# dpeerlab/segger

Hardware: AMD Instinct MI355X
Metric: edges scored/sec (tx->cell) fwd+bwd (higher is better)
Workload: dtype bf16; 1 GPU; C2: single Xenium-scale tile per GPU, 1000000 tx, 10000 nuclei, k=15 kNN (Ett=15000000, Etb=393796, Ep=2435646), training step fwd+bwd+Adam, attention dropout 0.2; parallelism=dp1

## Files before the change

include/segger_amd.h:

```cpp
#ifndef SEGGER_AMD_H
#define SEGGER_AMD_H

#include <stddef.h>
#include <stdint.h>

#ifdef __cplusplus
extern "C" {
#endif

#if defined(__GNUC__) || defined(__clang__)
#pragma GCC visibility push(default)
#endif

#define SEGGER_ABI_VERSION 32

enum segger_status {
  SEGGER_OK = 0,
  SEGGER_EINVAL = -1,
  SEGGER_EUNSUPPORTED = -2,
  SEGGER_EHIP = -3,
  SEGGER_EWORKSPACE = -4
};

enum segger_dtype { SEGGER_F32 = 0, SEGGER_BF16 = 1, SEGGER_F16 = 2 };
// ... 256 lines not shown
int segger_sample_negatives(const int64_t* pos, int64_t n, int64_t n_b, const int64_t* n_b_dev, uint64_t seed,
                            const uint64_t* seed_dev, int64_t* neg, segger_stream_t stream);

int segger_metric_fwd(const void* z, int64_t ld_z, int64_t n, int32_t channels, int32_t dtype, const int64_t* pos,
                      const int64_t* neg, const float* d_pos, const float* d_neg, const float* w, float eps,
                      float* loss, void* workspace, size_t workspace_bytes, segger_stream_t stream);
int segger_metric_bwd(const void* z, int64_t ld_z, int64_t n, int32_t channels, int32_t dtype, const int64_t* pos,
                      const int64_t* neg, const float* d_pos, const float* d_neg, const float* w, float eps,
                      const float* grad_scale_dev, float* grad_z, segger_stream_t stream);

size_t segger_triplet_workspace_bytes(int64_t n_edges);
int segger_triplet_fwd(const segger_triplet_args* args, segger_stream_t stream);
int segger_triplet_bwd(const segger_triplet_args* args, segger_stream_t stream);

#define SEGGER_LOSS_HEAD_DEFER_FINISH 1
typedef struct segger_loss_head_args {
  const void* z_tx; int64_t ld_ztx; int64_t n_tx;
  const void* z_bd; int64_t ld_zbd; int64_t n_bd;
  int32_t channels, dtype;
  const int64_t* tx_pos; const int64_t* tx_neg; float tx_margin, tx_eps;
  const int64_t* bd_pos; const int64_t* bd_neg; const float* bd_dpos; const float* bd_dneg; const float* bd_w; float bd_eps;
  int32_t sg_kind;
  const int64_t* sg_src; const int64_t* sg_pos; const int64_t* sg_neg; int64_t n_sg; float sg_margin, sg_eps;
  const int64_t* sg_pos_indptr; const int32_t* sg_pos_eid; const int32_t* sg_of_tx;
  const float* a; const float* b; const float* grad_out; float* out; float* grad_raw;
  float* tx_w; int32_t* tx_state; int32_t* tx_next; int32_t* tx_hot_id; float* tx_hot_acc;
  const void* y_tx; int64_t ld_ytx; float norm_eps; int32_t reserved_;
  void* grad_tx; int64_t ld_gtx; float* grad_bd;
  void* workspace; size_t workspace_bytes; int32_t* ticket;
} segger_loss_head_args;
size_t segger_loss_head_workspace_bytes(int64_t n_tx, int64_t n_bd, int64_t n_sg);
int64_t segger_loss_head_max_hot_rows(int64_t n_tx);
int segger_loss_head_supported(int32_t channels, int32_t dtype);
int segger_loss_head_fwd(const segger_loss_head_args* args, segger_stream_t stream);
int segger_loss_head_bwd(const segger_loss_head_args* args, segger_stream_t stream);

#define SEGGER_MINMAX_INITIALISED 1
#define SEGGER_MINMAX_KEEP_EMPTY 2
int segger_segment_minmax_ex(const float* pos, const int64_t* batch, int64_t n, int64_t n_graphs, float* mins, float* maxs,
                             int32_t flags, segger_stream_t stream);
int segger_segment_minmax(const float* pos, const int64_t* batch, int64_t n, int64_t n_graphs,
                          float* mins, float* maxs, segger_stream_t stream);

int segger_linear_supported(int32_t k_in, int32_t m_out, int32_t dtype);
int segger_linear_fwd(const void* x, int64_t ldx, const void* w, const float* bias, void* y, int64_t ldy,
                      int64_t n_rows, int32_t k_in, int32_t m_out, int32_t dtype, segger_stream_t stream);
int segger_linear_fwd_silu_grad(const void* x, int64_t ldx, const void* w, const void* gate, int64_t ld_gate, void* y,
// ... 277 lines not shown
```

segger_amd/_lib.py:

```python
from __future__ import annotations

import ctypes as C
import os
from typing import Optional

import torch

_HERE = os.path.dirname(os.path.abspath(__file__))
LIB_PATH = os.environ.get("SEGGER_AMD_LIB") or os.path.join(_HERE, "libsegger_amd.so")
ABI_VERSION = 32
THRESHOLDS_CHUNK = 1024
FEATURES_TILE, FEATURES_SLAB_ROWS, FEATURES_MAX_SLABS = 64, 512, 32
FEATURES_MAX_COLS, FEATURES_MAX_K = 32768, 256
KNN_BF_MAX_D, KNN_BF_MAX_K, KNN_BF_MAX_SLABS = 256, 64, 32
CONTAM_MAX_TYPES, CONTAM_MAX_K, CONTAM_MAX_REF_GENES, CONTAM_LDS_BYTES = 256, 64, 32768, 65536
MORPH_MAX_VERTS, MORPH_COLS, MORPH_ERR_OFFSETS, MORPH_ERR_CAP = 4096, 12, 1, 2
PJOIN_CONTAINS, PJOIN_INTERSECTS = 0, 1
PJOIN_ERR_OFFSETS, PJOIN_ERR_CAP, PJOIN_ERR_BUFFER, PJOIN_ERR_FILL = 1, 2, 4, 8
BOUNDARY_MAX_SMOOTHING, BOUNDARY_CHUNK_MAX_HULL, BOUNDARY_COUNTERS = 6, 2048, 8
OUTLINE_MAX_POINTS, OUTLINE_COUNTERS = 2048, 10

SEGGER_F32, SEGGER_BF16, SEGGER_F16 = 0, 1, 2
DTYPE_CODE = {torch.float32: SEGGER_F32, torch.bfloat16: SEGGER_BF16, torch.float16: SEGGER_F16}

# ... 147 lines not shown


class FrontJoinArgs(C.Structure):
    _fields_ = [
        ("table", vp), ("ids", vp), ("n_rows_table", C.c_int32), ("D", C.c_int32), ("dtype", C.c_int32), ("reserved_", C.c_int32),
        ("pe", vp), ("ld_pe", C.c_int64), ("n_tx", C.c_int64), ("n_bd", C.c_int64),
        ("xb", vp), ("ld_xb", C.c_int64),
        ("out_tx", vp), ("ld_out_tx", C.c_int64), ("out_bd", vp), ("ld_out_bd", C.c_int64),
        ("g_tx", vp), ("ld_g_tx", C.c_int64), ("g_bd", vp), ("ld_g_bd", C.c_int64),
        ("g_pe", vp), ("ld_g_pe", C.c_int64), ("g_xb", vp), ("ld_g_xb", C.c_int64),
        ("g_table", vp), ("gene_ptr", vp), ("gene_rows", vp), ("workspace", vp), ("workspace_bytes", C.c_size_t),
    ]


LOSS_HEAD_DEFER_FINISH = 1


class LossHeadArgs(C.Structure):
    _fields_ = [
        ("z_tx", vp), ("ld_ztx", C.c_int64), ("n_tx", C.c_int64),
        ("z_bd", vp), ("ld_zbd", C.c_int64), ("n_bd", C.c_int64),
        ("channels", C.c_int32), ("dtype", C.c_int32),
        ("tx_pos", vp), ("tx_neg", vp), ("tx_margin", C.c_float), ("tx_eps", C.c_float),
        ("bd_pos", vp), ("bd_neg", vp), ("bd_dpos", vp), ("bd_dneg", vp), ("bd_w", vp), ("bd_eps", C.c_float),
        ("sg_kind", C.c_int32),
        ("sg_src", vp), ("sg_pos", vp), ("sg_neg", vp), ("n_sg", C.c_int64), ("sg_margin", C.c_float), ("sg_eps", C.c_float),
        ("sg_pos_indptr", vp), ("sg_pos_eid", vp), ("sg_of_tx", vp),
        ("a", vp), ("b", vp), ("grad_out", vp), ("out", vp), ("grad_raw", vp),
        ("tx_w", vp), ("tx_state", vp), ("tx_next", vp), ("tx_hot_id", vp), ("tx_hot_acc", vp),
        ("y_tx", vp), ("ld_ytx", C.c_int64), ("norm_eps", C.c_float), ("reserved_", C.c_int32),
# ... 106 lines not shown
    "segger_front_join_fwd": (C.c_int, [C.POINTER(FrontJoinArgs), vp]),
    "segger_front_join_bwd": (C.c_int, [C.POINTER(FrontJoinArgs), vp]),
    "segger_embed_gelu_bwd_workspace_bytes": (C.c_size_t, [C.c_int64, C.c_int32, C.c_int32]),
    "segger_embed_gelu_bwd": (C.c_int, [vp, C.c_int64, vp, vp, C.c_int64, C.c_int64, C.c_int32, C.c_int32, vp, C.c_int64,
                                        vp, vp, vp, vp, C.c_size_t, C.c_int32, vp]),
    "segger_l2norm_fwd": (C.c_int, [vp, C.c_int64, C.c_int64, C.c_int32, C.c_float, vp, C.c_int64, C.c_int32, vp]),
    "segger_l2norm_bwd": (C.c_int, [vp, C.c_int64, vp, C.c_int64, C.c_int64, C.c_int32, C.c_float, vp, C.c_int64, C.c_int32, vp]),
    "segger_segment_rowsum_workspace_bytes": (C.c_size_t, [C.c_int64, C.c_int32, C.c_int32]),
    "segger_segment_rowsum": (C.c_int, [vp, C.c_int64, C.c_int64, C.c_int32, C.c_int32, vp, vp, C.c_int32, vp, vp,
                                        C.c_size_t, vp]),
    "segger_colsum_workspace_bytes": (C.c_size_t, [C.c_int64, C.c_int32]),
    "segger_colsum": (C.c_int, [vp, C.c_int64, C.c_int64, C.c_int32, C.c_int32, vp, vp, C.c_size_t, vp]),
    "segger_l2norm_many": (C.c_int, [C.POINTER(L2NormSeg), C.c_int32, C.c_int32, C.c_float, C.c_int32, vp]),
    "segger_loss_head_workspace_bytes": (C.c_size_t, [C.c_int64, C.c_int64, C.c_int64]),
    "segger_loss_head_max_hot_rows": (C.c_int64, [C.c_int64]),
    "segger_loss_head_supported": (C.c_int, [C.c_int32, C.c_int32]),
    "segger_loss_head_fwd": (C.c_int, [C.POINTER(LossHeadArgs), vp]),
    "segger_loss_head_bwd": (C.c_int, [C.POINTER(LossHeadArgs), vp]),
    "segger_knn_workspace_bytes": (C.c_size_t, [C.c_int64, C.c_int32, C.c_int32]),
    "segger_knn_grid": (C.c_int, [vp, C.c_int64, vp, C.c_int64, C.c_int32, C.c_float, C.c_float, C.c_float, C.c_float,
                                  C.c_int32, C.c_int32, vp, vp, vp, C.c_size_t, vp]),
    "segger_quadtree_workspace_bytes": (C.c_int64, [C.c_int64, C.c_int32, C.c_int64, C.c_int64]),
    "segger_quadtree_build": (C.c_int, [vp, C.c_int64, C.c_double, C.c_double, C.c_double, C.c_int32, C.c_int64, C.c_int64,
                                        vp, vp, vp, vp, vp, vp, vp, vp, C.c_size_t, vp]),
    "segger_quadtree_label": (C.c_int, [vp, C.c_int64, C.c_double, C.c_double, C.c_double, C.c_double, C.c_double, C.c_int32,
                                        vp, vp, vp, vp, C.c_int64, vp, vp]),
    "segger_assign_update": (C.c_int, [vp, vp, vp, vp, vp, C.c_int64, vp, vp, vp, vp, C.c_int64, vp]),
    "segger_assign_finalize": (C.c_int, [vp, C.c_int64, vp, vp, vp]),
    "segger_expression_workspace_bytes": (C.c_int64, [C.c_int64, C.c_int64, C.c_int64]),
    "segger_expression_build": (C.c_int, [vp, vp, vp, vp, vp, C.c_int64, C.c_int64, C.c_int64, vp, vp, vp, vp, vp, vp, vp, vp,
# ... 122 lines not shown
```

segger_amd/csrc/loss_head.hip:

```cpp
#include "common.h"
#include "post_common.h"

namespace segger {
namespace {

constexpr int kItemsPerBlock = 64;
constexpr int kChainCap = 64;
constexpr int32_t kOverflow = -2;

template <typename T, int CPL> struct Row;
template <int CPL> struct Row<float, CPL> {
  static __device__ __forceinline__ void load(const float* p, float (&f)[CPL]) {
    if constexpr (CPL == 2) { const float2 v = *reinterpret_cast<const float2*>(p); f[0] = v.x; f[1] = v.y; }
    else {
#pragma unroll
      for (int k = 0; k < CPL; k += 4) {
        const f32x4 v = *reinterpret_cast<const f32x4*>(p + k);
        f[k] = v.x; f[k + 1] = v.y; f[k + 2] = v.z; f[k + 3] = v.w;
      }
    }
  }
  static __device__ __forceinline__ void store(float* p, const float (&f)[CPL]) {
    if constexpr (CPL == 2) *reinterpret_cast<float2*>(p) = float2{f[0], f[1]};
    else {
// ... 37 lines not shown
  Vec8<f16_t>::unpack2(*reinterpret_cast<const uint32_t*>(p), a, b);
}

__device__ __forceinline__ float softplus_(float x) { return fmaxf(x, 0.f) + log1pf(__expf(-fabsf(x))); }
__device__ __forceinline__ float sigmoid_(float x) { return 1.0f / (1.0f + __expf(-x)); }

struct LossHeadParams {
  const void* ztx; int64_t ld_ztx; int64_t n_tx;
  const void* zbd; int64_t ld_zbd; int64_t n_bd;
  const int64_t* tx_pos; const int64_t* tx_neg; float tx_margin, tx_eps;
  const int64_t* bd_pos; const int64_t* bd_neg; const float* bd_dpos; const float* bd_dneg; const float* bd_w; float bd_eps;
  const int64_t* sg_src; const int64_t* sg_pos; const int64_t* sg_neg; int64_t n_sg; float sg_margin, sg_eps; int sg_kind;
  const int64_t* sg_indptr; const int32_t* sg_eid; const int32_t* sg_of_tx;
  const float* a; const float* b; const float* gout; float* out; float* graw;
  float* tx_w; int32_t* state; int32_t* next;
  int32_t* hot_id; float* hot_acc; int64_t max_hot;
  const void* ytx; int64_t ld_ytx; float norm_eps;
  void* gtx; int64_t ld_gtx; float* gbd;
  float* partial; int32_t* ticket;
  int nb_tx, nb_bd, nb_sg;
  int nb_sg_fin;
  int defer;
};

__device__ __forceinline__ float graw_of(const LossHeadParams& p, int i) {
  return p.defer ? (p.gout[3] * p.b[i] + p.gout[i]) * p.a[i] : p.graw[i];
}

template <typename T, int CPL>
__global__ __launch_bounds__(256) void loss_head_fwd_kernel(LossHeadParams p) {
// ... 21 lines not shown
      float sp = 0.f, sn = 0.f;
#pragma unroll
      for (int k = 0; k < CPL; ++k) {
        const float dp = a[k] - pp[k] + p.tx_eps, dn = a[k] - nn[k] + p.tx_eps;
        sp = fmaf(dp, dp, sp); sn = fmaf(dn, dn, sn);
      }
      sp = lane_block_sum<16>(sp); sn = lane_block_sum<16>(sn);
      const float dap = sqrtf(sp), dan = sqrtf(sn);
      const float l = dap - dan + p.tx_margin;
      if (ok && gl == 0) acc += fmaxf(l, 0.f);
      if (p.tx_w != nullptr && t < p.n_tx) {
        const bool active = ok && l > 0.f;
        const float wp = active && dap > 0.f ? 1.0f / dap : 0.f;
        const float wn = active && dan > 0.f ? 1.0f / dan : 0.f;
        if (gl < 2) {
          const float wk = gl == 0 ? wp : wn;
          const int64_t tgt = gl == 0 ? ip : in;
          const int32_t code = (int32_t)(2 * t + gl);
          p.tx_w[code] = wk;
          if (wk != 0.f) {
            const int32_t slot = atomicAdd(p.state + 2 * tgt + 1, 1);
            if (slot < kChainCap) {
              p.next[code] = atomicExch(p.state + 2 * tgt, code + 1);
            } else {
              p.next[code] = kOverflow;
              if (slot == kChainCap) {
                const int32_t hid = atomicAdd(p.state + 2 * p.n_tx, 1);
                if ((int64_t)hid < p.max_hot) {
                  float* acc_row = p.hot_acc + (int64_t)hid * C;
                  for (int k = 0; k < C; ++k) acc_row[k] = 0.f;
                  p.hot_id[p.n_tx + hid] = 0;
                  __threadfence();
                }
                p.hot_id[tgt] = hid;
              }
            }
          }
        }
      }
    }
  } else if (blk < p.nb_tx + p.nb_bd) {
    const int64_t base = (int64_t)(blk - p.nb_tx) * kItemsPerBlock;
#pragma unroll 1
    for (int q = wave * 4 + grp; q < kItemsPerBlock; q += 16) {
      const int64_t i = base + q;
      bool ok = i < p.n_bd;
      int64_t ip = ok ? p.bd_pos[i] : 0, in = ok ? p.bd_neg[i] : 0;
      const float w = ok ? p.bd_w[i] : 0.f;
      if ((uint64_t)ip >= (uint64_t)p.n_bd || (uint64_t)in >= (uint64_t)p.n_bd || w == 0.f) { ok = false; ip = in = 0; }
      const int64_t ii = ok ? i : 0;
      float x[CPL], yp[CPL], yn[CPL];
      Row<T, CPL>::load(zbd + ii * p.ld_zbd + c0, x);
// ... 98 lines not shown
__global__ __launch_bounds__(256) void loss_head_bwd_kernel(LossHeadParams p) {
  constexpr int C = 16 * CPL;
  const int lane = threadIdx.x & 63, wave = threadIdx.x >> 6;
  const int grp = lane >> 4, gl = lane & 15, c0 = gl * CPL;
  const int blk = blockIdx.x;
  const T* ztx = static_cast<const T*>(p.ztx);
  const T* zbd = static_cast<const T*>(p.zbd);
  if (p.defer && blk == p.nb_tx + p.nb_bd + p.nb_sg) {
    loss_head_finish_body(p);
    return;
  }
  if (blk < p.nb_tx) {
    const float sc_tx = p.n_tx > 0 ? graw_of(p, 0) / (float)p.n_tx : 0.f;
    const float sc_sg = p.n_sg > 0 ? graw_of(p, 2) * (p.sg_kind == SEGGER_LOSS_BCE ? 0.5f : 1.0f) / (float)p.n_sg : 0.f;
    const int64_t base = (int64_t)blk * kItemsPerBlock;
    auto finish_row = [&](int64_t row, float (&g)[CPL]) {
      if (p.ytx != nullptr) {
        float y[CPL];
        Row<T, CPL>::load(static_cast<const T*>(p.ytx) + row * p.ld_ytx + c0, y);
        float ss = 0.f;
#pragma unroll
        for (int k = 0; k < CPL; ++k) ss = fmaf(y[k], y[k], ss);
        const float nrm = sqrtf(lane_block_sum<16>(ss));
        const float inv = 1.0f / fmaxf(nrm, p.norm_eps);
        float dot = 0.f;
#pragma unroll
        for (int k = 0; k < CPL; ++k) dot = fmaf(y[k] * inv, g[k], dot);
        dot = lane_block_sum<16>(dot);
        if (nrm < p.norm_eps) dot = 0.f;
#pragma unroll
        for (int k = 0; k < CPL; ++k) g[k] = (g[k] - y[k] * inv * dot) * inv;
      }
      Row<T, CPL>::store(static_cast<T*>(p.gtx) + row * p.ld_gtx + c0, g);
    };
    auto hot_add = [&](int64_t row, const float (&g)[CPL]) {
      const int64_t hid = p.hot_id[row];
      if ((uint64_t)hid >= (uint64_t)p.max_hot) return;
      float* acc = p.hot_acc + hid * C + c0;
#pragma unroll
      for (int k = 0; k < CPL; ++k) atomicAdd(acc + k, g[k]);
      __threadfence();
      int32_t old = 0;
      if (gl == 0) old = atomicAdd(p.hot_id + p.n_tx + hid, 1);
      old = __shfl(old, lane & 48, 64);
      if (old == p.state[2 * row + 1] - kChainCap) {
        __threadfence();
        float t[CPL];
#pragma unroll
        for (int k = 0; k < CPL; ++k) t[k] = __hip_atomic_load(acc + k, __ATOMIC_RELAXED, __HIP_MEMORY_SCOPE_AGENT);
        finish_row(row, t);
      }
    };
#pragma unroll 1
    for (int i = wave * 4 + grp; i < kItemsPerBlock; i += 16) {
      const int64_t r = base + i;
      if (r >= p.n_tx) continue;
      float a[CPL], g[CPL];
      Row<T, CPL>::load(ztx + r * p.ld_ztx + c0, a);
#pragma unroll
      for (int k = 0; k < CPL; ++k) g[k] = 0.f;
      const float uwp = p.tx_w[2 * r], uwn = p.tx_w[2 * r + 1];
      const float wp = uwp * sc_tx, wn = uwn * sc_tx;
      if (uwp != 0.f || uwn != 0.f) {
        const int64_t ip = p.tx_pos[r], in = p.tx_neg[r];
        float pp[CPL], nn[CPL], dp[CPL], dn[CPL];
        Row<T, CPL>::load(ztx + ip * p.ld_ztx + c0, pp);
        Row<T, CPL>::load(ztx + in * p.ld_ztx + c0, nn);
#pragma unroll
        for (int k = 0; k < CPL; ++k) {
          dp[k] = (a[k] - pp[k] + p.tx_eps) * wp; dn[k] = (a[k] - nn[k] + p.tx_eps) * wn;
          g[k] += dp[k] - dn[k];
        }
        if (uwp != 0.f && p.next[2 * r] == kOverflow) {
#pragma unroll
          for (int k = 0; k < CPL; ++k) dp[k] = -dp[k];
          hot_add(ip, dp);
        }
        if (uwn != 0.f && p.next[2 * r + 1] == kOverflow) hot_add(in, dn);
      }
      const int32_t total = p.state[2 * r + 1];
      int32_t cur = p.state[2 * r];
#pragma unroll 1
      for (int it = 0; it < kChainCap && cur > 0 && (int64_t)cur <= 2 * p.n_tx; ++it) {
        const int32_t code = cur - 1;
        const int64_t t = code >> 1;
        const float w = p.tx_w[code] * sc_tx;
        const int32_t nxt = p.next[code];
        float at[CPL];
        Row<T, CPL>::load(ztx + t * p.ld_ztx + c0, at);
        const float sgn = (code & 1) ? w : -w;
#pragma unroll
        for (int k = 0; k < CPL; ++k) g[k] = fmaf(at[k] - a[k] + p.tx_eps, sgn, g[k]);
        cur = nxt;
      }
      if (p.sg_of_tx != nullptr && sc_sg != 0.f) {
        const int64_t e = p.sg_of_tx[r];
        if (e >= 0 && e < p.n_sg) {
          const int64_t j = p.sg_pos[e], jn = p.sg_neg[e];
          if (p.sg_src[e] == r && (uint64_t)j < (uint64_t)p.n_bd && (uint64_t)jn < (uint64_t)p.n_bd) {
            float pj[CPL], nv[CPL];
            Row<T, CPL>::load(zbd + j * p.ld_zbd + c0, pj);
            Row<T, CPL>::load(zbd + jn * p.ld_zbd + c0, nv);
            float s0 = 0.f, s1 = 0.f;
            if (p.sg_kind == SEGGER_LOSS_BCE) {
#pragma unroll
              for (int k = 0; k < CPL; ++k) { s0 = fmaf(a[k], pj[k], s0); s1 = fmaf(a[k], nv[k], s1); }
              s0 = lane_block_sum<16>(s0); s1 = lane_block_sum<16>(s1);
              const float dlp = (sigmoid_(s0) - 1.0f) * sc_sg, dln = sigmoid_(s1) * sc_sg;
#pragma unroll
              for (int k = 0; k < CPL; ++k) g[k] += dlp * pj[k] + dln * nv[k];
            } else {
              float dp[CPL], dn[CPL];
#pragma unroll
              for (int k = 0; k < CPL; ++k) {
                dp[k] = a[k] - pj[k] + p.sg_eps; dn[k] = a[k] - nv[k] + p.sg_eps;
                s0 = fmaf(dp[k], dp[k], s0); s1 = fmaf(dn[k], dn[k], s1);
              }
              s0 = lane_block_sum<16>(s0); s1 = lane_block_sum<16>(s1);
              const float dap = sqrtf(s0), dan = sqrtf(s1);
              if (dap - dan + p.sg_margin > 0.f) {
                const float ip_ = dap > 0.f ? sc_sg / dap : 0.f, in_ = dan > 0.f ? sc_sg / dan : 0.f;
#pragma unroll
                for (int k = 0; k < CPL; ++k) g[k] += dp[k] * ip_ - dn[k] * in_;
              }
            }
          }
        }
      }
      if (total > kChainCap) hot_add(r, g);
      else finish_row(r, g);
    }
  } else if (blk < p.nb_tx + p.nb_bd) {
    const float sc = graw_of(p, 1);
    const int64_t base = (int64_t)(blk - p.nb_tx) * kItemsPerBlock;
#pragma unroll 1
    for (int q = wave * 4 + grp; q < kItemsPerBlock; q += 16) {
      const int64_t i = base + q;
      if (i >= p.n_bd) continue;
      const int64_t ip = p.bd_pos[i], in = p.bd_neg[i];
      const float w = p.bd_w[i];
      if ((uint64_t)ip >= (uint64_t)p.n_bd || (uint64_t)in >= (uint64_t)p.n_bd || w == 0.f) continue;
      float x[CPL], yp[CPL], yn[CPL];
      Row<T, CPL>::load(zbd + i * p.ld_zbd + c0, x);
      Row<T, CPL>::load(zbd + ip * p.ld_zbd + c0, yp);
      Row<T, CPL>::load(zbd + in * p.ld_zbd + c0, yn);
// ... 119 lines not shown
  const int64_t nb_tx = blocks_of(a->n_tx), nb_bd = blocks_of(a->n_bd);
  const int64_t nb_sg = bwd ? (a->n_sg > 0 ? a->n_bd : 0) : blocks_of(a->n_sg);
  SEGGER_REQUIRE(nb_tx + nb_bd + nb_sg < 0x7fffffffLL, "segger_loss_head: too many blocks");
  const size_t need = segger_loss_head_workspace_bytes(a->n_tx, a->n_bd, a->n_sg);
  if (!a->workspace || a->workspace_bytes < need) return workspace_too_small("segger_loss_head", a->workspace_bytes, need);
  LossHeadParams p{};
  p.ztx = a->z_tx; p.ld_ztx = a->ld_ztx; p.n_tx = a->n_tx;
  p.zbd = a->z_bd; p.ld_zbd = a->ld_zbd; p.n_bd = a->n_bd;
  p.tx_pos = a->tx_pos; p.tx_neg = a->tx_neg; p.tx_margin = a->tx_margin; p.tx_eps = a->tx_eps;
  p.bd_pos = a->bd_pos; p.bd_neg = a->bd_neg; p.bd_dpos = a->bd_dpos; p.bd_dneg = a->bd_dneg; p.bd_w = a->bd_w; p.bd_eps = a->bd_eps;
  p.sg_src = a->sg_src; p.sg_pos = a->sg_pos; p.sg_neg = a->sg_neg; p.n_sg = a->n_sg;
  p.sg_margin = a->sg_margin; p.sg_eps = a->sg_eps; p.sg_kind = a->sg_kind;
  p.sg_indptr = a->sg_pos_indptr; p.sg_eid = a->sg_pos_eid; p.sg_of_tx = a->sg_of_tx;
  p.a = a->a; p.b = a->b; p.gout = a->grad_out; p.out = a->out; p.graw = a->grad_raw;
  p.tx_w = a->tx_w; p.state = a->tx_state; p.next = a->tx_next;
  p.hot_id = a->tx_hot_id; p.hot_acc = a->tx_hot_acc; p.max_hot = segger_loss_head_max_hot_rows(a->n_tx);
  p.ytx = a->y_tx; p.ld_ytx = a->ld_ytx; p.norm_eps = a->norm_eps;
  p.gtx = a->grad_tx; p.ld_gtx = a->ld_gtx; p.gbd = a->grad_bd;
  p.partial = static_cast<float*>(a->workspace); p.ticket = a->ticket;
  p.nb_tx = (int)nb_tx; p.nb_bd = (int)nb_bd; p.nb_sg = (int)nb_sg;
  p.defer = (a->reserved_ & SEGGER_LOSS_HEAD_DEFER_FINISH) ? 1 : 0;
  SEGGER_REQUIRE(!p.defer || a->grad_out, "segger_loss_head: DEFER_FINISH needs grad_out (the gradient the backward will receive)");
  p.nb_sg_fin = (int)blocks_of(a->n_sg);
  if (!bwd) {
    SEGGER_REQUIRE(!a->tx_w == !a->tx_state && !a->tx_state == !a->tx_next && !a->tx_next == !a->tx_hot_id && !a->tx_hot_id == !a->tx_hot_acc,
                   "segger_loss_head_fwd: tx_w, tx_state, tx_next, tx_hot_id and tx_hot_acc go together");
    SEGGER_REQUIRE(!a->grad_out || a->grad_raw, "segger_loss_head_fwd: grad_out needs grad_raw");
    SEGGER_REQUIRE(!a->grad_bd || is_aligned(a->grad_bd, 16), "segger_loss_head_fwd: grad_bd must be 16-byte aligned");
  } else {
    SEGGER_REQUIRE(a->grad_raw && a->tx_w && a->tx_state && a->tx_next && a->tx_hot_id && a->tx_hot_acc,
// ... 33 lines not shown
    SEGGER_LAUNCH_CHECK("loss_head_finish_kernel");
  }
  return SEGGER_OK;
}

}
}

using namespace segger;

extern "C" size_t segger_loss_head_workspace_bytes(int64_t n_tx, int64_t n_bd, int64_t n_sg) {
  const int64_t nb = blocks_of(n_tx > 0 ? n_tx : 0) + blocks_of(n_bd > 0 ? n_bd : 0) + blocks_of(n_sg > 0 ? n_sg : 0);
  return (size_t)(nb > 0 ? nb : 1) * sizeof(float) + 16;
}

extern "C" int64_t segger_loss_head_max_hot_rows(int64_t n_tx) { return n_tx > 0 ? 2 * n_tx / (kChainCap + 1) + 2 : 0; }

extern "C" int segger_loss_head_supported(int32_t channels, int32_t dtype) {
  return (channels == 32 || channels == 64 || channels == 128) && (dtype == SEGGER_F32 || dtype == SEGGER_BF16 || dtype == SEGGER_F16);
}

extern "C" int segger_loss_head_fwd(const segger_loss_head_args* a, segger_stream_t stream) {
  return launch<false>(a, (hipStream_t)stream);
}

extern "C" int segger_loss_head_bwd(const segger_loss_head_args* a, segger_stream_t stream) {
  return launch<true>(a, (hipStream_t)stream);
}
```

segger_amd/ops/__init__.py:

```python
from __future__ import annotations

import os



_FWD_PAIR = 1
_BWD_PAIR = 1

_CONTRIB_MIN_EDGES = 16384
ONE_LAUNCH_LOSS_HEAD = True
LOSS_HEAD_ONE_LAUNCH_MAX_ROWS = (1 << 30) - 2
USE_ANCHOR_ROWS = True

FUSED_WGRAD_DX = True
FUSED_GELU_GATE = True
F32_SPLIT = os.environ.get("SEGGER_AMD_F32_EXACT", "0") in ("", "0")
F32_GATE_EPILOGUE = True
F32_SPLIT_WGRAD = True
LINEAR_PAIR = True
WGRAD_PAIR = True

FUSED_POSMLP = True
FUSED_POSMLP_BWD = True
POS_POLY_F32 = True

# ... 30 lines not shown
```

segger_amd/ops/heads.py:

```python
from __future__ import annotations

from collections import namedtuple
import ctypes as C
from typing import Optional

import torch
from torch import Tensor

from .. import _lib
from .._lib import DTYPE_CODE
from ..graph import EdgeCSR
from .. import ops
from ._common import _prenorm_of, _rows


@torch.no_grad()
def edge_cos_argmax(by_src: EdgeCSR, z_src: Tensor, z_dst: Tensor, *, dst_index: Optional[Tensor] = None,
                    min_similarity: Optional[float] = None, eps: float = 1e-8, return_sim: bool = False):
    _lib.require_cuda(z_src, z_dst)
    lib = _lib.load()
    dev = z_src.device
    if z_src.dtype != z_dst.dtype or z_src.dtype not in DTYPE_CODE:
        raise TypeError("edge_cos_argmax: z_src / z_dst must share a supported dtype")
    c = int(z_src.shape[1])
# ... 303 lines not shown
def anchor_index(src: Tensor, n_rows: int) -> Tensor:
    inv = torch.full((int(n_rows),), -1, dtype=torch.int32, device=src.device)
    if src.numel():
        inv[src.long()] = torch.arange(src.numel(), dtype=torch.int32, device=src.device)
    return inv


def loss_head_fused_supported(z_tx: Tensor, z_bd: Tensor, spec: "LossHeadSpec") -> bool:
    n, c = int(z_tx.shape[0]), int(z_tx.shape[1])
    return (ops.ONE_LAUNCH_LOSS_HEAD and spec.tx_anchors_are_rows and z_tx.dtype in DTYPE_CODE and z_tx.dtype == z_bd.dtype
            and bool(_lib.load().segger_loss_head_supported(c, DTYPE_CODE[z_tx.dtype])) and int(z_bd.shape[1]) == c
            and 0 < n <= ops.LOSS_HEAD_ONE_LAUNCH_MAX_ROWS and spec.tx.anchors.numel() == n and z_bd.shape[0] > 0
            and (spec.sg is None or spec.sg.pos_groups is not None))


_FusedState = namedtuple("_FusedState", "tx_w head nxt gbd graw hot_acc out ws hint deferred")


def _loss_head_args(z_tx, z_bd, a, b, idx: _Indices, spec: LossHeadSpec, graw, ws, st: Optional[_FusedState]):
    tx, sg = spec.tx, spec.sg
    n_tx, c = int(z_tx.shape[0]), int(z_tx.shape[1])
    g = _lib.LossHeadArgs()
    g.z_tx, g.ld_ztx = _rows(z_tx, c, "z_tx")
    g.z_bd, g.ld_zbd = _rows(z_bd, c, "z_bd")
    g.n_tx, g.n_bd, g.channels, g.dtype = n_tx, int(z_bd.shape[0]), c, DTYPE_CODE[z_tx.dtype]
    g.tx_pos, g.tx_neg, g.tx_margin, g.tx_eps = idx.tx_pos.data_ptr(), idx.tx_neg.data_ptr(), float(tx.margin), float(tx.eps)
    g.bd_pos, g.bd_neg, g.bd_dpos, g.bd_dneg = (t.data_ptr() for t in (idx.bd_pos, idx.bd_neg, idx.bd_dpos, idx.bd_dneg))
    g.bd_w, g.bd_eps = idx.bd_w.data_ptr(), float(spec.bd.eps)
    g.sg_kind = _LOSS_KIND[spec.sg_kind]
    if sg is not None and idx.sg_src.numel():
        g.sg_src, g.sg_pos, g.sg_neg = idx.sg_src.data_ptr(), idx.sg_pos.data_ptr(), idx.sg_neg.data_ptr()
        g.n_sg = int(idx.sg_src.numel())
        g.sg_margin, g.sg_eps = float(sg.margin), float(sg.eps)
    g.a, g.b, g.grad_raw = a.data_ptr(), b.data_ptr(), graw.data_ptr()
    g.workspace, g.workspace_bytes, g.ticket = ws.data_ptr(), ws.numel(), _ticket(z_tx.device).data_ptr()
    if st is not None:
        g.tx_w, g.tx_state, g.tx_next, g.grad_bd = st.tx_w.data_ptr(), st.head.data_ptr(), st.nxt.data_ptr(), st.gbd.data_ptr()
        g.tx_hot_id, g.tx_hot_acc = st.nxt[2 * n_tx:].data_ptr(), st.hot_acc.data_ptr()
    return g


class _LossHeadFused(torch.autograd.Function):

    @staticmethod
    def forward(ctx, t_tx, t_bd, a, b, spec: LossHeadSpec, z_tx=None, z_bd=None, eps_tx=0.0, eps_bd=0.0):
        prenorm = z_tx is not None
        if not prenorm:
            z_tx, z_bd = t_tx, t_bd
        _lib.require_cuda(z_tx, z_bd, a, b)
        lib = _lib.load()
        dev = z_tx.device
        n_tx, c = int(z_tx.shape[0]), int(z_tx.shape[1])
        n_bd = int(z_bd.shape[0])
# ... 1 lines not shown
        a, b = _f32(a.detach()), _f32(b.detach())
        idx = _indices(spec, anchors=False)
        n_sg = int(idx.sg_src.numel()) if idx.sg_src is not None else 0
        out = torch.empty(4, dtype=torch.float32, device=dev)
        graw = torch.empty(3, dtype=torch.float32, device=dev)
        ws = torch.empty(lib.segger_loss_head_workspace_bytes(n_tx, n_bd, n_sg), dtype=torch.uint8, device=dev)
        st = None
        if need:
            tx_w = torch.empty((n_tx, 2), dtype=torch.float32, device=dev)
            head = spec.tx_state
            if head is None:
                head = torch.zeros(2 * n_tx + 4, dtype=torch.int32, device=dev)
            elif head.dtype != torch.int32 or head.numel() < 2 * n_tx + 4 or not head.is_contiguous():
                raise ValueError("loss_head: tx_state must be a contiguous int32 [2 n_tx + 4] tensor (zero-filled)")
            n_hot = int(lib.segger_loss_head_max_hot_rows(n_tx))
            nxt = torch.empty(2 * n_tx + n_tx + n_hot, dtype=torch.int32, device=dev)
            hot_acc = torch.empty((n_hot, c), dtype=torch.float32, device=dev)
            gbd = torch.empty((n_bd, c), dtype=torch.float32, device=dev)
            hint = spec.grad_out_hint
            if hint is not None:
                hint = hint.detach()
                if hint.dtype != torch.float32 or hint.numel() != 4 or not hint.is_contiguous() or hint.device != dev:
                    raise ValueError("loss_head: grad_out_hint must be a contiguous float32 [4] tensor on the embeddings' device")
            st = _FusedState(tx_w, head, nxt, gbd, graw, hot_acc, out, ws, hint, bool(hint is not None and spec.defer_finish))
        g = _loss_head_args(z_tx, z_bd, a, b, idx, spec, graw, ws, st)
        g.out = out.data_ptr()
        if st is not None and st.hint is not None:
            g.grad_out, g.reserved_ = st.hint.data_ptr(), (_lib.LOSS_HEAD_DEFER_FINISH if st.deferred else 0)
        with _lib.on_device(dev):
            rc = lib.segger_loss_head_fwd(C.byref(g), _lib.stream_ptr(dev))
        _lib.check(rc, "segger_loss_head_fwd")
        if need:
            ctx.save_for_backward(t_tx, t_bd, z_tx, z_bd, a, b, *idx)
            ctx.spec, ctx.state, ctx.prenorm, ctx.eps = spec, st, prenorm, (float(eps_tx), float(eps_bd))
        return out

    @staticmethod
    def backward(ctx, g_out):
        t_tx, t_bd, z_tx, z_bd, a, b, *idx = ctx.saved_tensors
        idx, spec, st, sg = _Indices(*idx), ctx.spec, ctx.state, ctx.spec.sg
        lib = _lib.load()
        dev, dt = z_tx.device, z_tx.dtype
        n_tx, c = int(z_tx.shape[0]), int(z_tx.shape[1])
        n_bd = int(z_bd.shape[0])
        if getattr(ctx, "_ran", False):
            st.gbd.zero_()
            st.hot_acc.zero_()
            st.nxt[3 * n_tx:].zero_()
        ctx._ran = True
        stream = _lib.stream_ptr(dev)
        g_out = g_out.detach().to(torch.float32).contiguous()
        hinted = st.hint is not None and g_out.data_ptr() == st.hint.data_ptr()
        n_sg = int(idx.sg_src.numel()) if sg is not None else 0
        uniq, of_tx = False, None
        if n_sg:
            uniq = _anchors_unique(sg.anchors_unique)
            if uniq:
                of_tx = spec.sg_of_tx() if callable(spec.sg_of_tx) else spec.sg_of_tx
                if of_tx is None:
                    of_tx = anchor_index(idx.sg_src, n_tx)
                if of_tx.dtype != torch.int32 or of_tx.numel() < n_tx or not of_tx.is_contiguous():
                    raise ValueError("loss_head: sg_of_tx must be a contiguous int32 [n_tx] tensor")
            pg = sg.pos_groups
            if pg.n_rows != n_bd or pg.n_edges != n_sg:
                raise ValueError("loss_head: pos_groups does not describe the segmentation triplets")
        fuse_norm = ctx.prenorm and (not n_sg or uniq)
        out_dummy = torch.empty(4, dtype=torch.float32, device=dev)
        if st.deferred and not hinted:
            raise RuntimeError("loss_head: defer_finish promised a backward with the hinted gradient")
        ws = st.ws if st.deferred else torch.empty(lib.segger_loss_head_workspace_bytes(n_tx, n_bd, n_sg), dtype=torch.uint8,
                                                   device=dev)
        g = _loss_head_args(z_tx, z_bd, a, b, idx, spec, st.graw, ws, st)
        g.out = out_dummy.data_ptr()
        if st.deferred:
            g.out, g.grad_out, g.reserved_ = st.out.data_ptr(), st.hint.data_ptr(), _lib.LOSS_HEAD_DEFER_FINISH
        if n_sg:
            g.sg_pos_indptr, g.sg_pos_eid = pg.indptr.data_ptr(), (pg.eid.data_ptr() if pg.n_edges else None)
            g.sg_of_tx = _lib.ptr(of_tx)
        gtx = torch.empty((n_tx, c), dtype=dt, device=dev)
        g.grad_tx, g.ld_gtx = gtx.data_ptr(), c
        if fuse_norm:
            g.y_tx, g.ld_ytx = _rows(t_tx, c, "y_tx")
            g.norm_eps = ctx.eps[0]
        with _lib.on_device(dev):
            if not hinted:
                _lib.check(lib.segger_loss_combine_bwd(g_out.data_ptr(), a.data_ptr(), b.data_ptr(), 3, st.graw.data_ptr(),
                                                       stream), "segger_loss_combine_bwd")
            _lib.check(lib.segger_loss_head_bwd(C.byref(g), stream), "segger_loss_head_bwd")
            if n_sg and not uniq:
                sa = _triplet_args(idx.sg_src, idx.sg_pos, idx.sg_neg, z_tx, z_bd, float(sg.margin), float(sg.eps), spec.sg_kind)
# ... 44 lines not shown
```

Measured before the change: 62.31 million edges/s.

## Store first incoming loss-head edges in per-row slots and prefetch row metadata

Replaces the linked-list chain for the first eight incoming tx triplet references per row with a fixed slot array, so the backward can gather them in parallel instead of chasing pointers serially. The overflow marker moves into the sign of tx_w, which removes a read of next[] for each row. Per-row metadata (weights, indices, state, segmentation edge) is now loaded one iteration ahead, and the pos, neg and y loads are issued together. The cost is extra memory for slots of n_tx*8 ints, new alignment requirements, and more registers.

```diff
diff --git a/include/segger_amd.h b/include/segger_amd.h
--- a/include/segger_amd.h
+++ b/include/segger_amd.h
@@ -294,6 +294,7 @@
 int segger_triplet_bwd(const segger_triplet_args* args, segger_stream_t stream);
 
 #define SEGGER_LOSS_HEAD_DEFER_FINISH 1
+#define SEGGER_LOSS_HEAD_SLOTS 2
 typedef struct segger_loss_head_args {
   const void* z_tx; int64_t ld_ztx; int64_t n_tx;
   const void* z_bd; int64_t ld_zbd; int64_t n_bd;
@@ -311,6 +312,7 @@
 } segger_loss_head_args;
 size_t segger_loss_head_workspace_bytes(int64_t n_tx, int64_t n_bd, int64_t n_sg);
 int64_t segger_loss_head_max_hot_rows(int64_t n_tx);
+int64_t segger_loss_head_next_words(int64_t n_tx);
 int segger_loss_head_supported(int32_t channels, int32_t dtype);
 int segger_loss_head_fwd(const segger_loss_head_args* args, segger_stream_t stream);
 int segger_loss_head_bwd(const segger_loss_head_args* args, segger_stream_t stream);
diff --git a/segger_amd/_lib.py b/segger_amd/_lib.py
--- a/segger_amd/_lib.py
+++ b/segger_amd/_lib.py
@@ -185,6 +185,7 @@
 
 
 LOSS_HEAD_DEFER_FINISH = 1
+LOSS_HEAD_SLOTS = 2
 
 
 class LossHeadArgs(C.Structure):
@@ -321,6 +322,7 @@
     "segger_l2norm_many": (C.c_int, [C.POINTER(L2NormSeg), C.c_int32, C.c_int32, C.c_float, C.c_int32, vp]),
     "segger_loss_head_workspace_bytes": (C.c_size_t, [C.c_int64, C.c_int64, C.c_int64]),
     "segger_loss_head_max_hot_rows": (C.c_int64, [C.c_int64]),
+    "segger_loss_head_next_words": (C.c_int64, [C.c_int64]),
     "segger_loss_head_supported": (C.c_int, [C.c_int32, C.c_int32]),
     "segger_loss_head_fwd": (C.c_int, [C.POINTER(LossHeadArgs), vp]),
     "segger_loss_head_bwd": (C.c_int, [C.POINTER(LossHeadArgs), vp]),
diff --git a/segger_amd/csrc/loss_head.hip b/segger_amd/csrc/loss_head.hip
--- a/segger_amd/csrc/loss_head.hip
+++ b/segger_amd/csrc/loss_head.hip
@@ -6,7 +6,7 @@
 
 constexpr int kItemsPerBlock = 64;
 constexpr int kChainCap = 64;
-constexpr int32_t kOverflow = -2;
+constexpr int kSlots = 8;
 
 template <typename T, int CPL> struct Row;
 template <int CPL> struct Row<float, CPL> {
@@ -75,6 +75,7 @@
   const int64_t* sg_indptr; const int32_t* sg_eid; const int32_t* sg_of_tx;
   const float* a; const float* b; const float* gout; float* out; float* graw;
   float* tx_w; int32_t* state; int32_t* next;
+  int32_t* slots;
   int32_t* hot_id; float* hot_acc; int64_t max_hot;
   const void* ytx; int64_t ld_ytx; float norm_eps;
   void* gtx; int64_t ld_gtx; float* gbd;
@@ -126,16 +127,18 @@
         const float wp = active && dap > 0.f ? 1.0f / dap : 0.f;
         const float wn = active && dan > 0.f ? 1.0f / dan : 0.f;
         if (gl < 2) {
-          const float wk = gl == 0 ? wp : wn;
+          float wk = gl == 0 ? wp : wn;
           const int64_t tgt = gl == 0 ? ip : in;
           const int32_t code = (int32_t)(2 * t + gl);
-          p.tx_w[code] = wk;
           if (wk != 0.f) {
+            const int32_t n_slots = p.slots != nullptr ? kSlots : 0;
             const int32_t slot = atomicAdd(p.state + 2 * tgt + 1, 1);
-            if (slot < kChainCap) {
+            if (slot < n_slots) {
+              p.slots[tgt * kSlots + slot] = code + 1;
+            } else if (slot < kChainCap) {
               p.next[code] = atomicExch(p.state + 2 * tgt, code + 1);
             } else {
-              p.next[code] = kOverflow;
+              wk = -wk;
               if (slot == kChainCap) {
                 const int32_t hid = atomicAdd(p.state + 2 * p.n_tx, 1);
                 if ((int64_t)hid < p.max_hot) {
@@ -148,6 +151,7 @@
               }
             }
           }
+          p.tx_w[code] = wk;
         }
       }
     }
@@ -276,10 +280,9 @@
     const float sc_tx = p.n_tx > 0 ? graw_of(p, 0) / (float)p.n_tx : 0.f;
     const float sc_sg = p.n_sg > 0 ? graw_of(p, 2) * (p.sg_kind == SEGGER_LOSS_BCE ? 0.5f : 1.0f) / (float)p.n_sg : 0.f;
     const int64_t base = (int64_t)blk * kItemsPerBlock;
-    auto finish_row = [&](int64_t row, float (&g)[CPL]) {
-      if (p.ytx != nullptr) {
-        float y[CPL];
-        Row<T, CPL>::load(static_cast<const T*>(p.ytx) + row * p.ld_ytx + c0, y);
+    const T* ytx = static_cast<const T*>(p.ytx);
+    auto finish_row = [&](int64_t row, float (&g)[CPL], const float (&y)[CPL]) {
+      if (ytx != nullptr) {
         float ss = 0.f;
 #pragma unroll
         for (int k = 0; k < CPL; ++k) ss = fmaf(y[k], y[k], ss);
@@ -307,46 +310,96 @@
       old = __shfl(old, lane & 48, 64);
       if (old == p.state[2 * row + 1] - kChainCap) {
         __threadfence();
-        float t[CPL];
+        float t[CPL], y[CPL];
+        if (ytx != nullptr) Row<T, CPL>::load(ytx + row * p.ld_ytx + c0, y);
 #pragma unroll
         for (int k = 0; k < CPL; ++k) t[k] = __hip_atomic_load(acc + k, __ATOMIC_RELAXED, __HIP_MEMORY_SCOPE_AGENT);
-        finish_row(row, t);
+        finish_row(row, t, y);
       }
     };
+    const bool sg_on = p.sg_of_tx != nullptr && sc_sg != 0.f && p.n_bd > 0;
+    const int32_t n_slots = p.slots != nullptr ? kSlots : 0;
+    struct RowWords { float2 w; int64_t ip, in; int2 st; int32_t e, slot; };
+    auto row_words = [&](int64_t r) {
+      RowWords x;
+      x.w = *reinterpret_cast<const float2*>(p.tx_w + 2 * r);
+      x.ip = p.tx_pos[r]; x.in = p.tx_neg[r];
+      x.st = *reinterpret_cast<const int2*>(p.state + 2 * r);
+      x.e = sg_on ? p.sg_of_tx[r] : -1;
+      x.slot = n_slots ? p.slots[r * kSlots + (gl & (kSlots - 1))] : 0;
+      return x;
+    };
+    auto add_slots = [&](const RowWords& x, int first, int32_t n_listed, const float (&a)[CPL], float (&g)[CPL]) {
+      constexpr int NB = kSlots / 2;
+      float w[NB], at[NB][CPL];
+      bool use[NB];
+      int32_t code[NB];
+#pragma unroll
+      for (int q = 0; q < NB; ++q) {
+        const int32_t c = __shfl(x.slot, (lane & 48) + first + q, 64);
+        use[q] = first + q < n_listed && c > 0 && (int64_t)c <= 2 * p.n_tx;
+        code[q] = use[q] ? c - 1 : 0;
+        w[q] = p.tx_w[code[q]];
+        Row<T, CPL>::load(ztx + (int64_t)(code[q] >> 1) * p.ld_ztx + c0, at[q]);
+      }
+#pragma unroll
+      for (int q = 0; q < NB; ++q) {
+        const float ws = fabsf(w[q]) * sc_tx;
+        const float sgn = (code[q] & 1) ? ws : -ws;
+#pragma unroll
+        for (int k = 0; k < CPL; ++k) g[k] = use[q] ? fmaf(at[q][k] - a[k] + p.tx_eps, sgn, g[k]) : g[k];
+      }
+    };
+    const int i0 = wave * 4 + grp;
+    RowWords ahead{};
+    if (base + i0 < p.n_tx) ahead = row_words(base + i0);
 #pragma unroll 1
-    for (int i = wave * 4 + grp; i < kItemsPerBlock; i += 16) {
+    for (int i = i0; i < kItemsPerBlock; i += 16) {
       const int64_t r = base + i;
-      if (r >= p.n_tx) continue;
-      float a[CPL], g[CPL];
+      if (r >= p.n_tx) break;
+      const RowWords x = ahead;
+      if (i + 16 < kItemsPerBlock && r + 16 < p.n_tx) ahead = row_words(r + 16);
+      const float uwp = x.w.x, uwn = x.w.y;
+      const bool own = (uwp != 0.f || uwn != 0.f) && (uint64_t)x.ip < (uint64_t)p.n_tx && (uint64_t)x.in < (uint64_t)p.n_tx;
+      const int64_t ip = own ? x.ip : 0, in = own ? x.in : 0;
+      const int32_t total = x.st.y;
+      const int32_t n_listed = total < n_slots ? (total > 0 ? total : 0) : n_slots;
+      float a[CPL], g[CPL], pp[CPL], nn[CPL], y[CPL];
       Row<T, CPL>::load(ztx + r * p.ld_ztx + c0, a);
+      Row<T, CPL>::load(ztx + ip * p.ld_ztx + c0, pp);
+      Row<T, CPL>::load(ztx + in * p.ld_ztx + c0, nn);
+      if (ytx != nullptr) Row<T, CPL>::load(ytx + r * p.ld_ytx + c0, y);
+      const bool has_e = sg_on && x.e >= 0 && (int64_t)x.e < p.n_sg;
+      int64_t j = 0, jn = 0, e_src = -1;
+      if (sg_on) {
+        const int64_t e = has_e ? x.e : 0;
+        e_src = p.sg_src[e]; j = p.sg_pos[e]; jn = p.sg_neg[e];
+      }
 #pragma unroll
       for (int k = 0; k < CPL; ++k) g[k] = 0.f;
-      const float uwp = p.tx_w[2 * r], uwn = p.tx_w[2 * r + 1];
-      const float wp = uwp * sc_tx, wn = uwn * sc_tx;
-      if (uwp != 0.f || uwn != 0.f) {
-        const int64_t ip = p.tx_pos[r], in = p.tx_neg[r];
-        float pp[CPL], nn[CPL], dp[CPL], dn[CPL];
-        Row<T, CPL>::load(ztx + ip * p.ld_ztx + c0, pp);
-        Row<T, CPL>::load(ztx + in * p.ld_ztx + c0, nn);
+      if (own) {
+        const float wp = fabsf(uwp) * sc_tx, wn = fabsf(uwn) * sc_tx;
+        float dp[CPL], dn[CPL];
 #pragma unroll
         for (int k = 0; k < CPL; ++k) {
           dp[k] = (a[k] - pp[k] + p.tx_eps) * wp; dn[k] = (a[k] - nn[k] + p.tx_eps) * wn;
           g[k] += dp[k] - dn[k];
         }
-        if (uwp != 0.f && p.next[2 * r] == kOverflow) {
+        if (uwp < 0.f) {
 #pragma unroll
           for (int k = 0; k < CPL; ++k) dp[k] = -dp[k];
           hot_add(ip, dp);
         }
-        if (uwn != 0.f && p.next[2 * r + 1] == kOverflow) hot_add(in, dn);
-      }
-      const int32_t total = p.state[2 * r + 1];
-      int32_t cur = p.state[2 * r];
+        if (uwn < 0.f) hot_add(in, dn);
+      }
+      if (n_listed > 0) add_slots(x, 0, n_listed, a, g);
+      if (n_listed > kSlots / 2) add_slots(x, kSlots / 2, n_listed, a, g);
+      int32_t cur = x.st.x;
 #pragma unroll 1
-      for (int it = 0; it < kChainCap && cur > 0 && (int64_t)cur <= 2 * p.n_tx; ++it) {
+      for (int it = 0; it < kChainCap - n_slots && cur > 0 && (int64_t)cur <= 2 * p.n_tx; ++it) {
         const int32_t code = cur - 1;
         const int64_t t = code >> 1;
-        const float w = p.tx_w[code] * sc_tx;
+        const float w = fabsf(p.tx_w[code]) * sc_tx;
         const int32_t nxt = p.next[code];
         float at[CPL];
         Row<T, CPL>::load(ztx + t * p.ld_ztx + c0, at);
@@ -355,42 +408,36 @@
         for (int k = 0; k < CPL; ++k) g[k] = fmaf(at[k] - a[k] + p.tx_eps, sgn, g[k]);
         cur = nxt;
       }
-      if (p.sg_of_tx != nullptr && sc_sg != 0.f) {
-        const int64_t e = p.sg_of_tx[r];
-        if (e >= 0 && e < p.n_sg) {
-          const int64_t j = p.sg_pos[e], jn = p.sg_neg[e];
-          if (p.sg_src[e] == r && (uint64_t)j < (uint64_t)p.n_bd && (uint64_t)jn < (uint64_t)p.n_bd) {
-            float pj[CPL], nv[CPL];
-            Row<T, CPL>::load(zbd + j * p.ld_zbd + c0, pj);
-            Row<T, CPL>::load(zbd + jn * p.ld_zbd + c0, nv);
-            float s0 = 0.f, s1 = 0.f;
-            if (p.sg_kind == SEGGER_LOSS_BCE) {
-#pragma unroll
-              for (int k = 0; k < CPL; ++k) { s0 = fmaf(a[k], pj[k], s0); s1 = fmaf(a[k], nv[k], s1); }
-              s0 = lane_block_sum<16>(s0); s1 = lane_block_sum<16>(s1);
-              const float dlp = (sigmoid_(s0) - 1.0f) * sc_sg, dln = sigmoid_(s1) * sc_sg;
-#pragma unroll
-              for (int k = 0; k < CPL; ++k) g[k] += dlp * pj[k] + dln * nv[k];
-            } else {
-              float dp[CPL], dn[CPL];
-#pragma unroll
-              for (int k = 0; k < CPL; ++k) {
-                dp[k] = a[k] - pj[k] + p.sg_eps; dn[k] = a[k] - nv[k] + p.sg_eps;
-                s0 = fmaf(dp[k], dp[k], s0); s1 = fmaf(dn[k], dn[k], s1);
-              }
-              s0 = lane_block_sum<16>(s0); s1 = lane_block_sum<16>(s1);
-              const float dap = sqrtf(s0), dan = sqrtf(s1);
-              if (dap - dan + p.sg_margin > 0.f) {
-                const float ip_ = dap > 0.f ? sc_sg / dap : 0.f, in_ = dan > 0.f ? sc_sg / dan : 0.f;
-#pragma unroll
-                for (int k = 0; k < CPL; ++k) g[k] += dp[k] * ip_ - dn[k] * in_;
-              }
-            }
+      if (has_e && e_src == r && (uint64_t)j < (uint64_t)p.n_bd && (uint64_t)jn < (uint64_t)p.n_bd) {
+        float pj[CPL], nv[CPL];
+        Row<T, CPL>::load(zbd + j * p.ld_zbd + c0, pj);
+        Row<T, CPL>::load(zbd + jn * p.ld_zbd + c0, nv);
+        float s0 = 0.f, s1 = 0.f;
+        if (p.sg_kind == SEGGER_LOSS_BCE) {
+#pragma unroll
+          for (int k = 0; k < CPL; ++k) { s0 = fmaf(a[k], pj[k], s0); s1 = fmaf(a[k], nv[k], s1); }
+          s0 = lane_block_sum<16>(s0); s1 = lane_block_sum<16>(s1);
+          const float dlp = (sigmoid_(s0) - 1.0f) * sc_sg, dln = sigmoid_(s1) * sc_sg;
+#pragma unroll
+          for (int k = 0; k < CPL; ++k) g[k] += dlp * pj[k] + dln * nv[k];
+        } else {
+          float dp[CPL], dn[CPL];
+#pragma unroll
+          for (int k = 0; k < CPL; ++k) {
+            dp[k] = a[k] - pj[k] + p.sg_eps; dn[k] = a[k] - nv[k] + p.sg_eps;
+            s0 = fmaf(dp[k], dp[k], s0); s1 = fmaf(dn[k], dn[k], s1);
           }
+          s0 = lane_block_sum<16>(s0); s1 = lane_block_sum<16>(s1);
+          const float dap = sqrtf(s0), dan = sqrtf(s1);
+          if (dap - dan + p.sg_margin > 0.f) {
+            const float ip_ = dap > 0.f ? sc_sg / dap : 0.f, in_ = dan > 0.f ? sc_sg / dan : 0.f;
+#pragma unroll
+            for (int k = 0; k < CPL; ++k) g[k] += dp[k] * ip_ - dn[k] * in_;
+          }
         }
       }
       if (total > kChainCap) hot_add(r, g);
-      else finish_row(r, g);
+      else finish_row(r, g, y);
     }
   } else if (blk < p.nb_tx + p.nb_bd) {
     const float sc = graw_of(p, 1);
@@ -540,6 +587,11 @@
   p.sg_indptr = a->sg_pos_indptr; p.sg_eid = a->sg_pos_eid; p.sg_of_tx = a->sg_of_tx;
   p.a = a->a; p.b = a->b; p.gout = a->grad_out; p.out = a->out; p.graw = a->grad_raw;
   p.tx_w = a->tx_w; p.state = a->tx_state; p.next = a->tx_next;
+  if ((a->reserved_ & SEGGER_LOSS_HEAD_SLOTS) && a->tx_next != nullptr) {
+    SEGGER_REQUIRE(((uintptr_t)a->tx_next % 32) == 0, "segger_loss_head: with SEGGER_LOSS_HEAD_SLOTS tx_next must be 32-byte aligned");
+    p.slots = a->tx_next + (segger_loss_head_next_words(a->n_tx) - (int64_t)kSlots * a->n_tx);
+  }
+  SEGGER_REQUIRE(((uintptr_t)a->tx_w % 8) == 0 && ((uintptr_t)a->tx_state % 8) == 0, "segger_loss_head: tx_w / tx_state must be 8-byte aligned");
   p.hot_id = a->tx_hot_id; p.hot_acc = a->tx_hot_acc; p.max_hot = segger_loss_head_max_hot_rows(a->n_tx);
   p.ytx = a->y_tx; p.ld_ytx = a->ld_ytx; p.norm_eps = a->norm_eps;
   p.gtx = a->grad_tx; p.ld_gtx = a->ld_gtx; p.gbd = a->grad_bd;
@@ -603,6 +655,10 @@
   return (size_t)(nb > 0 ? nb : 1) * sizeof(float) + 16;
 }
 
+extern "C" int64_t segger_loss_head_next_words(int64_t n_tx) {
+  return n_tx > 0 ? ((2 * n_tx + 7) & ~(int64_t)7) + (int64_t)kSlots * n_tx : 0;
+}
+
 extern "C" int64_t segger_loss_head_max_hot_rows(int64_t n_tx) { return n_tx > 0 ? 2 * n_tx / (kChainCap + 1) + 2 : 0; }
 
 extern "C" int segger_loss_head_supported(int32_t channels, int32_t dtype) {
diff --git a/segger_amd/ops/__init__.py b/segger_amd/ops/__init__.py
--- a/segger_amd/ops/__init__.py
+++ b/segger_amd/ops/__init__.py
@@ -9,6 +9,7 @@
 
 _CONTRIB_MIN_EDGES = 16384
 ONE_LAUNCH_LOSS_HEAD = True
+LOSS_HEAD_SLOTS = True
 LOSS_HEAD_ONE_LAUNCH_MAX_ROWS = (1 << 30) - 2
 USE_ANCHOR_ROWS = True
 
diff --git a/segger_amd/ops/heads.py b/segger_amd/ops/heads.py
--- a/segger_amd/ops/heads.py
+++ b/segger_amd/ops/heads.py
@@ -341,7 +341,7 @@
             and (spec.sg is None or spec.sg.pos_groups is not None))
 
 
-_FusedState = namedtuple("_FusedState", "tx_w head nxt gbd graw hot_acc out ws hint deferred")
+_FusedState = namedtuple("_FusedState", "tx_w head nxt hot_id slots gbd graw hot_acc out ws hint deferred")
 
 
 def _loss_head_args(z_tx, z_bd, a, b, idx: _Indices, spec: LossHeadSpec, graw, ws, st: Optional[_FusedState]):
@@ -363,7 +363,8 @@
     g.workspace, g.workspace_bytes, g.ticket = ws.data_ptr(), ws.numel(), _ticket(z_tx.device).data_ptr()
     if st is not None:
         g.tx_w, g.tx_state, g.tx_next, g.grad_bd = st.tx_w.data_ptr(), st.head.data_ptr(), st.nxt.data_ptr(), st.gbd.data_ptr()
-        g.tx_hot_id, g.tx_hot_acc = st.nxt[2 * n_tx:].data_ptr(), st.hot_acc.data_ptr()
+        g.tx_hot_id, g.tx_hot_acc = st.hot_id.data_ptr(), st.hot_acc.data_ptr()
+        g.reserved_ = _lib.LOSS_HEAD_SLOTS if st.slots else 0
     return g
 
 
@@ -395,7 +396,9 @@
             elif head.dtype != torch.int32 or head.numel() < 2 * n_tx + 4 or not head.is_contiguous():
                 raise ValueError("loss_head: tx_state must be a contiguous int32 [2 n_tx + 4] tensor (zero-filled)")
             n_hot = int(lib.segger_loss_head_max_hot_rows(n_tx))
-            nxt = torch.empty(2 * n_tx + n_tx + n_hot, dtype=torch.int32, device=dev)
+            slots = bool(ops.LOSS_HEAD_SLOTS)
+            n_next = int(lib.segger_loss_head_next_words(n_tx)) if slots else 2 * n_tx
+            nxt = torch.empty(n_next + n_tx + n_hot, dtype=torch.int32, device=dev)
             hot_acc = torch.empty((n_hot, c), dtype=torch.float32, device=dev)
             gbd = torch.empty((n_bd, c), dtype=torch.float32, device=dev)
             hint = spec.grad_out_hint
@@ -403,11 +406,13 @@
                 hint = hint.detach()
                 if hint.dtype != torch.float32 or hint.numel() != 4 or not hint.is_contiguous() or hint.device != dev:
                     raise ValueError("loss_head: grad_out_hint must be a contiguous float32 [4] tensor on the embeddings' device")
-            st = _FusedState(tx_w, head, nxt, gbd, graw, hot_acc, out, ws, hint, bool(hint is not None and spec.defer_finish))
+            st = _FusedState(tx_w, head, nxt, nxt[n_next:], slots, gbd, graw, hot_acc, out, ws, hint,
+                             bool(hint is not None and spec.defer_finish))
         g = _loss_head_args(z_tx, z_bd, a, b, idx, spec, graw, ws, st)
         g.out = out.data_ptr()
         if st is not None and st.hint is not None:
-            g.grad_out, g.reserved_ = st.hint.data_ptr(), (_lib.LOSS_HEAD_DEFER_FINISH if st.deferred else 0)
+            g.grad_out = st.hint.data_ptr()
+            g.reserved_ |= _lib.LOSS_HEAD_DEFER_FINISH if st.deferred else 0
         with _lib.on_device(dev):
             rc = lib.segger_loss_head_fwd(C.byref(g), _lib.stream_ptr(dev))
         _lib.check(rc, "segger_loss_head_fwd")
@@ -427,7 +432,7 @@
         if getattr(ctx, "_ran", False):
             st.gbd.zero_()
             st.hot_acc.zero_()
-            st.nxt[3 * n_tx:].zero_()
+            st.hot_id[n_tx:].zero_()
         ctx._ran = True
         stream = _lib.stream_ptr(dev)
         g_out = g_out.detach().to(torch.float32).contiguous()
@@ -454,7 +459,8 @@
         g = _loss_head_args(z_tx, z_bd, a, b, idx, spec, st.graw, ws, st)
         g.out = out_dummy.data_ptr()
         if st.deferred:
-            g.out, g.grad_out, g.reserved_ = st.out.data_ptr(), st.hint.data_ptr(), _lib.LOSS_HEAD_DEFER_FINISH
+            g.out, g.grad_out = st.out.data_ptr(), st.hint.data_ptr()
+            g.reserved_ |= _lib.LOSS_HEAD_DEFER_FINISH
         if n_sg:
             g.sg_pos_indptr, g.sg_pos_eid = pg.indptr.data_ptr(), (pg.eid.data_ptr() if pg.n_edges else None)
             g.sg_of_tx = _lib.ptr(of_tx)
```

New measurement: 62.86 million edges/s, median of 6. About the same (+0.9%).
